# millardjn/rusty_sr

Measured on AMD Instinct MI355X. Metric: output megapixels/sec at 3x upscale (BASELINE '4x'; reference factor is hard-wired 3), higher is better.
Workload: dtype f32

## Files before the change

rusty_sr_amd/csrc/sr_api.cpp:

```cpp
#include <hip/hip_runtime.h>

#include <algorithm>
#include <cmath>
#include <cstdio>
#include <cstdlib>
#include <chrono>
#include <cstring>
#include <new>
#include <string>
#include <thread>
#include <vector>

#include "../../include/srhip.h"
#include "../../include/srhip_experimental.h"
#include "sr_kernels.h"
#include "sr_internal.h"

namespace {

struct ParamLayout {
    size_t conv0, f_bias, f_activ, exp_bias, l_bias[3], l_activ[3], conv1, conv2, conv3, conv5, conv6, conv7, conv8,
        conv9, conv10, end;
    int E;
    explicit ParamLayout(int f) {
// ... 54 lines not shown
                                const int rr = c / 8, h = (c / 4) % 2, e = c % 4;
                                dst[base + (size_t)(2 * ts + rr) * 256 + (h * 32 + j) * 4 + e] = src[c];
                            } else {
                                _Float16 hi, lo;
                                split_half_host(src[c], hi, lo);
                                const int h = c / 8, e = c % 8;
                                hp[ts * 512 + (h * 32 + j) * 8 + e] = hi;
                                hp[1024 + ts * 512 + (h * 32 + j) * 8 + e] = lo;
                            }
                        }
                    }
                }
            }
}

void pack_steps_h16(std::vector<float>& dst, const float* w, int ks) {
    const int nt = ks * ks, np = (nt - 1) / 2;
    auto chunk = [&](int tap_a, int half_a, int tap_b, int half_b) {
        const size_t base = dst.size();
        dst.resize(base + kChunk, 0.0f);
        _Float16* hp = (_Float16*)(dst.data() + base);
        for (int ch = 0; ch < 2; ++ch)
            for (int lane = 0; lane < 64; ++lane) {
                const int g = lane >> 4, o = 16 * ch + (lane & 15);
                const int t = (g >> 1) ? tap_b : tap_a, half = (g >> 1) ? half_b : half_a;
                const int tap = (t % ks) * ks + t / ks;
                for (int e = 0; e < 8; ++e) {
                    _Float16 hi, lo;
                    split_half_host(w[((size_t)o * nt + tap) * 32 + 16 * half + 8 * (g & 1) + e], hi, lo);
                    hp[(ch * 64 + lane) * 8 + e] = hi;
// ... 143 lines not shown
    if (!out) return SR_E_INVALID;
    *out = nullptr;
    if (graph != SR_GRAPH_SR_NET && graph != SR_GRAPH_BILINEAR && graph != SR_GRAPH_DOWNSAMPLE) return SR_E_INVALID;
    if (graph == SR_GRAPH_SR_NET ? (factor < 2 || factor > 4) : factor != SR_FACTOR) return SR_E_FACTOR;
    if (n_params != (graph == SR_GRAPH_SR_NET ? ParamLayout(factor).end : 0)) return SR_E_PARAM_COUNT;
    if (graph == SR_GRAPH_SR_NET && !params) return SR_E_INVALID;
    int ndev = 0;
    if (hipGetDeviceCount(&ndev) != hipSuccess || ndev <= 0) return SR_E_NO_DEVICE;
    if (device < 0 || device >= ndev) return SR_E_INVALID;
    sr_ctx* c = new (std::nothrow) sr_ctx();
    if (!c) return SR_E_NOMEM;
    sr_device_guard restore_device;
    c->device = device;
    c->graph = graph;
    c->factor = factor;
    static const char* const kSwitch[12][2] = {{"th", "SRHIP_TH"}, {"pipe", "SRHIP_PIPE"}, {"bw", "SRHIP_BW"}, {"tail", "SRHIP_TAIL"},
                                               {"bands", "SRHIP_BANDS"}, {"geo", "SRHIP_GEO"}, {"rows", "SRHIP_ROWS"}, {"fork", "SRHIP_FORK"},
                                               {"forkshare", "SRHIP_FORKSHARE"}, {"forkmin", "SRHIP_FORKMIN"}, {"forktune", "SRHIP_FORKTUNE"}, {"halo", "SRHIP_HALO"}};
    for (const auto& sw : kSwitch)
        if (const char* e = getenv(sw[1])) (void)sr_set_experiment(c, sw[0], e);
    {
        unsigned long long hsh = 1469598103934665603ull;
        const unsigned char* pb = (const unsigned char*)params;
        for (size_t i = 0; i < n_params * sizeof(float); ++i) { hsh ^= pb[i]; hsh *= 1099511628211ull; }
        c->params_hash = hsh;
    }
    const bool trace = getenv("SRHIP_TRACE") != nullptr;
    auto t_last = std::chrono::steady_clock::now();
    auto mark = [&](const char* what) {
        if (!trace) return;
        const auto now = std::chrono::steady_clock::now();
// ... 43 lines not shown
            auto conv = [&](const float* wp, int ks) { if (h16) pack_steps_h16(w, wp, ks); else pack_steps(w, wp, ks, 1, split != 0, ident); };
            auto exp3 = [&](const float* wp) { pack_steps(w, wp, 3, expand_tiles(factor), split != 0, expand); };
            size_t* off = split ? c->off_wh : c->off_w;
            w.clear(); conv(params + L.conv1, 5);
            off[1] = push(w);
            w.clear(); conv(params + L.conv2, 5); conv(params + L.conv5, 3);
            off[2] = push(w);
            w.clear(); conv(params + L.conv3, 5); conv(params + L.conv6, 3); conv(params + L.conv8, 3);
            off[3] = push(w);
            w.clear();
            exp3(params + L.conv7); exp3(params + L.conv9); exp3(params + L.conv10);
            if (split) pack_lin_split(w, factor);
            else pack_lin(w, factor);
            off[4] = push(w);
        }
        const size_t boff[4] = {L.f_bias, L.l_bias[0], L.l_bias[1], L.l_bias[2]};
        const size_t aoff[4] = {L.f_activ, L.l_activ[0], L.l_activ[1], L.l_activ[2]};
        for (int s = 0; s < 4; ++s) c->off_bias[s] = push(vec32(boff[s], 32));
        for (int s = 0; s < 4; ++s) c->off_beta[s] = push(vec32(aoff[s], 32));
        {
            std::vector<float> eb((size_t)expand_tiles(factor) * 32, 0.0f);
            for (int nt = 0; nt < expand_tiles(factor); ++nt)
                for (int j = 0; j < 32; ++j) {
                    const int ch = expand_channel(factor, nt, j);
                    if (ch >= 0) eb[nt * 32 + j] = params[L.exp_bias + ch];
                }
            c->off_bias[4] = push(eb);
        }
        for (size_t k = L.conv1; k < L.end && c->split_ok; ++k) c->split_ok = std::fabs(params[k]) < 65504.0f;
        for (size_t k = L.conv0; k < L.conv0 + 2400 && c->split_ok; ++k) c->split_ok = std::fabs(params[k]) < 65504.0f;
// ... 89 lines not shown
    } else if (!strcmp(key, "tail")) {
        c->env_tail = *v ? (float)atof(v) : -1.0f;
    } else if (!strcmp(key, "fork")) {
        c->env_fork = *v ? atoi(v) : -1;
    } else if (!strcmp(key, "forkshare")) {
        c->fork_share = *v ? std::min(0.9, std::max(0.1, atof(v))) : 0.5;
    } else if (!strcmp(key, "forkmin")) {
        c->fork_min_rounds = *v ? atof(v) : 3.5;
    } else if (!strcmp(key, "forktune")) {
        c->fork_autotune = strcmp(v, "0") != 0;
        sr_device_guard restore_device;
        (void)hipSetDevice(c->device);
        sr_fork_tune_clear(c);
    } else if (!strcmp(key, "halo")) {
        c->layer_halos = !strcmp(v, "layers");
    } else if (!strcmp(key, "bw")) {
        c->env_bw = *v ? atoi(v) : -1;
    } else {
        return SR_E_INVALID;
    }
    return SR_OK;
}

int sr_get_experiment(sr_ctx* c, const char* key, char* buf, size_t cap) {
    if (!c || !key || !buf || cap == 0) return SR_E_INVALID;
    std::string out;
    if (!strcmp(key, "forktune")) {
        char line[160];
        for (const auto& t : c->fork_tune) {
            snprintf(line, sizeof line, "%dx%d+%d+%d %s %s %s %.4f %.4f\n", t.H, t.W, t.top, t.bot, t.precision == SR_PRECISION_F32 ? "f32" : "split_f16",
// ... 121 lines not shown
int StackJob::prepare() {
    static const int margin[5] = {5, 3, 2, 1, 0};
    tiles_x = (W + 31) / 32;
    const int rc = ensure_features(c, *ws, n, H, W, tiles_x, s);
    if (rc != SR_OK) return rc;
    const int cus = c->cus > 0 ? c->cus : 256;
    const int resident = 2 * cus;
    const bool planar = c->precision == SR_PRECISION_SPLIT_F16;
    for (int k = 0; k < 4; ++k) feat[k] = ws->d_feat[k] + (planar ? (size_t)kFeatPad * ws->pitch * 32 + kFeatPad * 4 : ((size_t)kFeatPad * ws->pitch + kFeatPad) * 32);
    for (int st = 0; st < 5; ++st) {
        Launch& l = L[st];
        l.y0 = layers ? top : std::max(0, top - margin[st]);
        l.y1 = layers ? bot : std::min(H, bot + margin[st]);
        const int rows = l.y1 - l.y0;
        const long tiles8 = (long)n * tiles_x * ((rows + 7) / 8);
        const int forced = (st == 4 && c->factor == 4 && c->precision == SR_PRECISION_SPLIT_F16) ? 4 : c->env_th[st];
        const bool small_launch = tiles8 < 2L * resident;
        const bool split = c->precision == SR_PRECISION_SPLIT_F16;
        const bool one_small_round = small_launch && (long)n * tiles_x * ((rows + 3) / 4) <= resident;
        l.pipe = st > 0 && c->env_pipe != 0 && (c->env_pipe == 2 || !small_launch || split || (st >= 2 && one_small_round));
        l.ty8 = (rows + 7) / 8; l.ty4 = 0;
        if (forced == 4 || (!forced && small_launch && (!split || tiles8 < cus))) {
            l.ty8 = 0; l.ty4 = (rows + 3) / 4;
        } else if (!forced && l.pipe && !small_launch) {
            const double rounds = (double)tiles8 / resident;
            float tail = c->env_tail;
            if (tail < 0.0f) tail = (!split && rounds >= 3.0 && !forked && st != 4) ? 1.0f : 0.0f;
            if (tail > 0.0f) {
                const long per_row = (long)n * tiles_x;
                const int want = (int)((tail * resident + per_row - 1) / per_row);
                l.ty8 = std::max(0, (rows - 4 * want) / 8);
                l.ty4 = std::max(0, (rows - 8 * l.ty8 + 3) / 4);
            }
        }
        if (!forced && l.pipe && !small_launch && !split && l.ty4 == 0 && (double)tiles8 / resident >= 3.0 && rows % 8 >= 1 && rows % 8 <= 4) {
            l.ty8 = rows / 8; l.ty4 = 1;
        }
// ... 46 lines not shown
        HIPCHK(c, hipStreamWaitEvent(s, gate->ready, 0));
        if (mark && gate->mark[1]) HIPCHK(c, hipEventRecord(gate->mark[1], s));
        if (lo >= hi) return rows(y0, y1);
        rc = rows(y0, lo);
        return rc != SR_OK ? rc : rows(hi, y1);
    }
    StageArgs a{};
    float* f = feat[0]; float* l1 = feat[1]; float* l2 = feat[2]; float* l3 = feat[3];
    a.pitch = ws->pitch; a.img_stride = ws->img_stride;
    switch (st) {
        case 1: a.src[0] = f; a.dst = l1; break;
        case 2: a.src[0] = f; a.src[1] = l1; a.dst = l2; break;
        case 3: a.src[0] = f; a.src[1] = l1; a.src[2] = l2; a.dst = l3; break;
        case 4: a.src[0] = l1; a.src[1] = l2; a.src[2] = l3; a.img = d_img; a.out = d_out; break;
    }
    a.wpack = P + (c->precision ? c->off_wh[st] : c->off_w[st]); a.bias = P + c->off_bias[st];
    a.beta = st < 4 ? P + c->off_beta[st] : nullptr;
    a.H = H; a.W = W; a.img_ch = img_ch;
    a.y_begin = y0; a.y_end = y1; a.tiles_x = tiles_x;
    a.n_img = n; a.queue = ws->d_queue + st * 8; a.domain = c->d_domain;
    a.grid[0] = make_tile_grid(8, y0, l.ty8, tiles_x, n, bw);
    a.grid[1] = make_tile_grid(4, y0 + 8 * l.ty8, l.ty4, tiles_x, n, bw);
    if (l.pipe) HIPCHK(c, sr_launch_stage_pipe(st, c->factor, a, c->precision, l.grid, img_u8, out_u8, s));
    else HIPCHK(c, sr_launch_stage(st, c->factor, a, l.th, c->precision, l.grid, img_u8, out_u8, s));
    return SR_OK;
}

}

int sr_run_stack(sr_ctx* c, const void* d_img, bool img_u8, int img_ch, int n, int H, int W, int halo_top,
                 int halo_bot, void* d_out, bool out_u8, hipStream_t s, int slot, const sr_halo_gate* gate) {
    if (!c || !d_img || !d_out || slot < 0 || slot > 1) return SR_E_INVALID;
    sr_device_guard restore_device;
    if (n <= 0 || H <= 0 || W <= 0) return SR_E_INVALID;
    if (img_u8 && img_ch != 3 && img_ch != 4) return SR_E_INVALID;
    if (c->graph != SR_GRAPH_SR_NET) {
        if (halo_top || halo_bot || gate) return SR_E_INVALID;
        if (c->graph == SR_GRAPH_DOWNSAMPLE && (H < 3 || W < 3)) return SR_E_INVALID;
        if (img_u8 != out_u8) return SR_E_INVALID;
// ... 744 lines not shown
```

rusty_sr_amd/csrc/sr_internal.h:

```cpp
#pragma once
#include <hip/hip_runtime.h>

#include <cstdint>
#include <string>
#include <utility>
#include <vector>

#include "../../include/srhip.h"

struct sr_ctx {
    int device = 0;
    int cus = 0, clock_mhz = 0;
    char name[128] = {0};
    hipStream_t stream = nullptr;
    float* d_params = nullptr;
    void* d_qtab = nullptr;
    size_t off_w0 = 0, off_w0h = 0, off_w[5] = {0}, off_wh[5] = {0}, off_bias[5] = {0}, off_beta[5] = {0};
    int precision = 0;
    bool split_ok = true;
    int* h_domain = nullptr;
    int* d_domain = nullptr;
    int domain_fallbacks = 0;
    bool dev_fault = false;
    int graph = SR_GRAPH_SR_NET;
    int factor = SR_FACTOR;
    struct Workspace {
        float* d_feat[4] = {nullptr, nullptr, nullptr, nullptr};
        size_t feat_cap_px = 0;
        int geo_n = 0, geo_h = 0, geo_w = 0;
        int pitch = 0; long img_stride = 0;
        int* d_queue = nullptr;
    } ws[2];
// ... 153 lines not shown
```

rusty_sr_amd/csrc/sr_kernels.h:

```cpp
#pragma once
#include <hip/hip_runtime.h>
#include <stdint.h>

struct TileDiv {
    uint32_t m, s;
};
inline TileDiv make_tile_div(uint32_t d) {
    TileDiv r{1u, 0u};
    while ((1u << r.s) < d) ++r.s;
    r.m = (uint32_t)(((uint64_t)1 << 32) * (((uint64_t)1 << r.s) - d) / d + 1);
    return r;
}

struct Conv0Args {
    const void* img;
    const float* wpack;
    const void* wpack_split;
    const float* bias;
    const float* beta;
    float* dst;
    int H, W, img_ch;
    int pitch;
    long img_stride;
    int y_begin, y_end;
// ... 59 lines not shown
    long total_px;
};
hipError_t sr_launch_clear_borders(const ClearArgs& a, hipStream_t s);

struct AuxArgs {
    const void* img;
    void* out;
    int n, H, W, img_ch;
    const void* qtab;
};
hipError_t sr_aux_build_tables(void** d_tab);
hipError_t sr_launch_aux(int graph, const AuxArgs& a, bool img_u8, bool out_u8, hipStream_t s);

hipError_t sr_launch_conv0(const Conv0Args& a, int th, int prec, int nblk, bool img_u8, hipStream_t s);
hipError_t sr_launch_stage(int stage, int factor, const StageArgs& a, int th, int prec, int nblk, bool img_u8, bool out_u8,
                           hipStream_t s);
hipError_t sr_launch_stage_pipe(int stage, int factor, const StageArgs& a, int prec, int grid, bool img_u8, bool out_u8,
                                hipStream_t s);
```

rusty_sr_amd/csrc/sr_kernels.hip:

```cpp
#include <hip/hip_runtime.h>
#include <stddef.h>
#include <stdint.h>

#include <mutex>
#include <set>
#include <type_traits>
#include <utility>

#include "sr_kernels.h"

#pragma clang fp contract(off)

typedef float f32x2 __attribute__((ext_vector_type(2)));
struct f32p { float x, y; };
__device__ __forceinline__ f32p operator+(f32p a, f32p b) { return f32p{a.x + b.x, a.y + b.y}; }
__device__ __forceinline__ f32p operator-(f32p a, f32p b) { return f32p{a.x - b.x, a.y - b.y}; }
__device__ __forceinline__ f32p operator*(f32p a, f32p b) { return f32p{a.x * b.x, a.y * b.y}; }
__device__ __forceinline__ f32p p_fma(f32p a, f32p b, f32p c) { return f32p{__builtin_fmaf(a.x, b.x, c.x), __builtin_fmaf(a.y, b.y, c.y)}; }
__device__ __forceinline__ void store_map8(char* p, uint32_t a, uint32_t b) { *(uint2*)p = make_uint2(a, b); }
typedef float f32x4 __attribute__((ext_vector_type(4)));
typedef float f32x16 __attribute__((ext_vector_type(16)));
typedef _Float16 f16x8 __attribute__((ext_vector_type(8)));
typedef _Float16 f16x2 __attribute__((ext_vector_type(2)));

// ... 498 lines not shown
                __builtin_amdgcn_sched_barrier(0);
                mfma(cur, nt);
                __builtin_amdgcn_sched_barrier(0);
                cur = nxt;
            }
        }
        const bool last = p == NP - 1 && nt == NTN - 1;
        sm.template end_step<0>(last);
        if (!last) load(nxt, nt + 1 < NTN ? p : p + 1, 0, sm.slot());
        if (((p * NTN + nt) * 4 + 3) % NTN == 0) sm.piece(((p * NTN + nt) * 4 + 3) / NTN);
        __builtin_amdgcn_sched_barrier(0);
        mfma(cur, nt);
        __builtin_amdgcn_sched_barrier(0);
        cur = nxt;
      }
    }
}

template <int TWH, int PS, int LO, int KS, int T, int NTN, typename Stream>
__device__ __forceinline__ void half_steps_h(f32x16 (&accm)[NTN * T], f32x16 (&accx)[NTN * T], const char* hb, const char* ring,
                                             Stream& sm, int wave, int lane) {
    constexpr int NT = KS * KS, NP = (NT + 1) / 2;
    const int i = lane & 31, h = lane >> 5;
    const int wlane = (h * 32 + i) * 16;
    const char* abase = hb + h * PS + ((wave * T) * TWH + i) * 16;
    struct Ops { f16x8 bh[2], bl[2], ah[2][T], al[2][T]; };
    auto row_id = [](int p, int ts, int m) {
        const int t = 2 * p + ts;
        return t < NT ? (t / KS) * 16 + (t % KS) + m : -1;
    };
// ... 428 lines not shown
                        for (int r = 0; r < 16; r += 2) {
                            uint32_t p0, p1;
                            quant2(r, p0, p1);
                            const int row0 = (r & 3) + 8 * (r >> 2);
                            if (writer && x0 + 4 * h + row0 < a.W) base[row0 * FACTOR] = p0;
                            if (writer && x0 + 4 * h + row0 + 1 < a.W) base[(row0 + 1) * FACTOR] = p1;
                        }
                    }
                }
            }
        }
    }
    return stores;
}

template <int N>
struct __attribute__((packed, aligned(4))) DwordRun { uint32_t w[N]; };
template <int N>
__device__ __forceinline__ void store_run_n(char* o, const uint32_t* w) {
    DwordRun<N> r;
#pragma unroll
    for (int k = 0; k < N; ++k) r.w[k] = w[k];
    *(DwordRun<N>*)o = r;
}
__device__ __forceinline__ void store_run_dwords(char* o, const uint32_t* w, int n) {
    if (n == 1) store_run_n<1>(o, w);
    else if (n == 2) store_run_n<2>(o, w);
    else if (n == 3) store_run_n<3>(o, w);
    else if (n == 4) store_run_n<4>(o, w);
    else if (n == 6) store_run_n<6>(o, w);
// ... 176 lines not shown
__device__ __forceinline__ int queue_slot(int x, int nbig, int nsmall, int idx) {
    int start, count;
    run_of_xcd(x, nbig, start, count);
    if (idx < count) return start + idx;
    idx -= count;
    run_of_xcd(x, nsmall, start, count);
    return idx < count ? nbig + start + idx : -1;
}
__device__ __forceinline__ int queue_total(int x, int nbig, int nsmall) {
    int start, cb, cs;
    run_of_xcd(x, nbig, start, cb);
    run_of_xcd(x, nsmall, start, cs);
    return cb + cs;
}
__device__ __forceinline__ int queue_first(int block, int nbig, int nsmall) { return queue_slot(block & 7, nbig, nsmall, block >> 3); }
template <int TH, int NSRC, int KS0, bool FINAL, bool IMG_U8, bool OUT_U8, int PREC, int FACTOR = 3>
__global__ __launch_bounds__(256, 2) void conv_stage_kernel(StageArgs a) {
    __builtin_amdgcn_s_setprio(3);
    constexpr int NW = 4, T = TH / NW;
    constexpr int NTN = FINAL ? (FACTOR * FACTOR + 9) / 10 : 1;
    using G0 = TileGeom<TH, KS0>;
    extern __shared__ __attribute__((aligned(16))) char smem[];
    char* tile = smem;
    char* ring = smem + 8 * G0::PLANE;

    const int tid = threadIdx.x, lane = tid & 63;
    const int wave = __builtin_amdgcn_readfirstlane(tid >> 6);
    const int i = lane & 31;
    constexpr bool H16 = kH16<PREC, FINAL>;
    constexpr int NTAPS = H16 ? KS0 * KS0 + (NSRC - 1) * 9
                              : 2 * ((KS0 * KS0 + 1) / 2 + (NSRC - 1) * 5) * NTN;
    const TileGrid& grid = a.grid[TH == 8 ? 0 : 1];
    float bias[NTN];
#pragma unroll
    for (int nt = 0; nt < NTN; ++nt) bias[nt] = a.bias[nt * 32 + i];
    const float beta = FINAL ? 0.f : a.beta[i];

    TileOffsets<TH, KS0, NW> off0;
    TileOffsets<TH, 3, NW> off3;
    off0.template init<PREC>(a.pitch, wave, lane);
    if constexpr (NSRC >= 2) off3.template init<PREC>(a.pitch, wave, lane);
    int n, tx, ty;
    tile_coords(grid, a.tiles_x, xcd_remap(blockIdx.x, gridDim.x), n, tx, ty);
    const int x0 = tx * kTW, y0 = grid.y0 + ty * TH;
#pragma unroll
// ... 9 lines not shown
            if constexpr (PREC == 1) accx[m][r] = 0.f;
        }
    f32x4 qm[H16 ? T : 1][2][2], qx[H16 ? T : 1][2][2];
    f32x4 bias2[2], beta2[2];
    if constexpr (H16) {
#pragma unroll
        for (int ch = 0; ch < 2; ++ch) {
            bias2[ch] = *(const f32x4*)(a.bias + 16 * ch + 4 * (lane >> 4));
            beta2[ch] = *(const f32x4*)(a.beta + 16 * ch + 4 * (lane >> 4));
        }
#pragma unroll
        for (int m = 0; m < T; ++m)
#pragma unroll
            for (int k = 0; k < 4; ++k) { qm[m][k >> 1][k & 1] = bias2[k & 1]; qx[m][k >> 1][k & 1] = f32x4{0.f, 0.f, 0.f, 0.f}; }
    }
    int gtap = 0, slot = 0;
    auto taps = [&](auto ks_tag) {
        constexpr int KS = decltype(ks_tag)::value;
        if constexpr (H16) source_steps_h16<TH, KS, T>(qm, qx, tile, ring, a.wpack, gtap, slot, NTAPS, wave, lane);
        else source_steps<TH, KS, T, NTN, PREC>(acc, accx, tile, ring, a.wpack, gtap, slot, NTAPS, wave, lane);
    };
    ring_barrier<0>();
    __builtin_amdgcn_s_setprio(0);
    taps(std::integral_constant<int, KS0>{});
    if constexpr (NSRC >= 2) {
        __builtin_amdgcn_s_setprio(3);
        stage_tile<TH, 3, PREC, NW>(tile, a.src[1], off3, a.img_stride, a.pitch, n, y0, x0, wave, lane);
        ring_barrier<0>();
        __builtin_amdgcn_s_setprio(0);
        taps(std::integral_constant<int, 3>{});
    }
    if constexpr (NSRC >= 3) {
        __builtin_amdgcn_s_setprio(3);
        stage_tile<TH, 3, PREC, NW>(tile, a.src[2], off3, a.img_stride, a.pitch, n, y0, x0, wave, lane);
        ring_barrier<0>();
        __builtin_amdgcn_s_setprio(0);
        taps(std::integral_constant<int, 3>{});
    }
    __builtin_amdgcn_s_setprio(3);
    if constexpr (FINAL)
        lin_taps<TH, T, IMG_U8, NW * 64, NTN, PREC, FACTOR>(acc, accx, tile, ring, a, a.wpack + (size_t)NTAPS * kChunkFloats, n, y0, x0, wave, lane, tid);
    uint32_t dom = 0;
    if constexpr (H16) {
        stage_epilogue_h16<T>(a, qm, qx, beta2, n, x0, y0, wave, lane, dom);
    } else if constexpr (FINAL && PREC == 1) {
        f32x4 fbias[NTN][4];
#pragma unroll
        for (int nt = 0; nt < NTN; ++nt)
#pragma unroll
            for (int k = 0; k < 4; ++k) fbias[nt][k] = *(const f32x4*)(a.bias + 32 * nt + 16 * (lane >> 5) + 4 * k);
        stage_epilogue_final_t<T, NTN, OUT_U8, FACTOR>(a, acc, accx, fbias, n, x0, y0, wave, lane);
    } else {
        static_assert(PREC == 0, "the split-half mode's tiles have epilogues of their own");
        stage_epilogue<TH, T, NTN, FINAL, OUT_U8, FACTOR>(a, acc, bias, beta, n, x0, y0, wave, lane);
    }
    if constexpr (PREC == 1 && !FINAL) domain_report(dom, a.domain);
}

// ... 260 lines not shown
    }
    __device__ __forceinline__ void piece(int g) {
        if (g < HalfTile<KSN>::G::NG && g < rq.ng) {
            htn.stage_one(g, rq.origin, rq.dst);
            st.tile_seq = ++st.issued;
        }
    }
    __device__ __forceinline__ int slot() const { return st.slot; }
    template <int EXTRA> __device__ __forceinline__ void end_step(bool last) {
        if (last) last_step_hook();
        if (last && mailbox) queue_publish(a, xcd, wave, lane, st, qs, mailbox);
        step_advance<EXTRA>(st, last, PREC == 1 && gs0 + step_no <= kRingAhead);
    }
};

template <int NSRC, int KS0, bool FINAL, bool IMG_U8, bool OUT_U8, int PREC, int FACTOR = 3>
__global__ __launch_bounds__(256, 2) void conv_stage_pipe_kernel(StageArgs a) {
    __builtin_amdgcn_s_setprio(3);
    constexpr int NTN = FINAL ? (FACTOR * FACTOR + 9) / 10 : 1;
    using H0 = HalfTile<KS0>;
    using H3 = HalfTile<3>;
    constexpr int HB = H0::BYTES;
    constexpr int NH = 2 * NSRC;
    constexpr bool H16 = kH16<PREC, FINAL>;
    constexpr int NSTEPS = H16 ? KS0 * KS0 + (NSRC - 1) * 9
                               : 2 * (H0::STEPS + (NSRC - 1) * H3::STEPS) * NTN;
    extern __shared__ __attribute__((aligned(16))) char smem[];
    char* ring = smem + 2 * HB;
    volatile int* s_next = (volatile int*)(ring + kRingBytes);
    float* s_wlin = (float*)(ring + kRingBytes + 16);
    float* s_lut = s_wlin + 9 * NTN * 128;
    constexpr bool kLinOwn = FINAL && NTN == 1;
    float* s_xown = s_lut + 256;
    const uint32_t lds0 = lds_addr(smem);

    const int tid = threadIdx.x, lane = tid & 63;
    const int wave = __builtin_amdgcn_readfirstlane(tid >> 6);
    const int i = lane & 31;
    const int nbig = a.grid[0].ntiles, nsmall = a.grid[1].ntiles;
    const int xcd = blockIdx.x & 7;
// ... 85 lines not shown
        f32x4 qm[H16 ? T : 1][2][2], qx[H16 ? T : 1][2][2];
        if constexpr (H16) {
#pragma unroll
            for (int m = 0; m < T; ++m)
#pragma unroll
                for (int k = 0; k < 4; ++k) { qm[m][k >> 1][k & 1] = bias2[k & 1]; qx[m][k >> 1][k & 1] = f32x4{0.f, 0.f, 0.f, 0.f}; }
        }
        constexpr bool QUAD = FINAL && PREC == 0 && T == 2;
        QuadAcc qa[QUAD ? NTN : 1];
        if constexpr (QUAD) {
#pragma unroll
            for (int nt = 0; nt < NTN; ++nt)
#pragma unroll
                for (int g = 0; g < 8; ++g) qa[nt][g] = f32x4{0.f, 0.f, 0.f, 0.f};
        }
        QueueState qs{0u, 0u, 0, 0, -1};
        if (!single) queue_pull_async(a, xcd, wave, lane, st, qs);
        st.have_next = false;
        LinPrefetch<IMG_U8, TH> linpx;
        auto do_half = [&](auto jc) {
            constexpr int j = decltype(jc)::value;
            constexpr int src = j >> 1;
            constexpr int KSJ = src == 0 ? KS0 : 3;
            constexpr int KSN = (j + 1 < NH) ? (((j + 1) >> 1) == 0 ? KS0 : 3) : KS0;
            const uint32_t other = lds0 + ((j + 1) & 1) * HB;
            const char* hb = smem + (j & 1) * HB;
            if constexpr (j == 1) {
                const int next = single ? -1 : __builtin_amdgcn_readfirstlane(*s_next);
                st.have_next = next >= 0;
                if (st.have_next) coords(next, nn, nx0, ny0, nsmall_tile);
            }
            HalfRequest rq;
            if constexpr (j + 1 < NH)
                rq = HalfRequest{T == 2 ? HalfTile<KSN>::G::NG : HalfTile<KSN>::NG_SMALL,
                                 HalfTile<KSN>::template origin_of<PREC>(a.src[(j + 1) >> 1], (j + 1) & 1, a.img_stride, a.pitch, n, y0, x0, wave),
                                 HalfTile<KSN>::plane_of(other, wave)};
            else
                rq = HalfRequest{!st.have_next ? 0 : nsmall_tile ? HalfTile<KSN>::NG_SMALL : HalfTile<KSN>::G::NG,
                                 HalfTile<KSN>::template origin_of<PREC>(a.src[0], 0, a.img_stride, a.pitch, nn, ny0, nx0, wave),
                                 HalfTile<KSN>::plane_of(other, wave)};
            if constexpr (FINAL && j == (kLinOwn ? NH - 2 : NH - 1)) linpx.issue(a, n, y0, x0, tid, st);
            const HalfTile<KSN>* htn;
            if constexpr (KSN == KS0) htn = (const HalfTile<KSN>*)&h0; else htn = (const HalfTile<KSN>*)&h3;
            using GJ = TileGeom<8, KSJ>;
            constexpr int PAIRS_J = (KSJ * KSJ - 1) / 2;
            constexpr int STEPS_J = H16 ? PAIRS_J + (j & 1) : HalfTile<KSJ>::STEPS * NTN;
            constexpr int GS0 = H16 ? (src == 0 ? 0 : KS0 * KS0 + (src - 1) * 9) + (j & 1) * PAIRS_J
                                    : (j == 0 ? 0 : j == 1 ? H0::STEPS : 2 * H0::STEPS + (j - 2) * H3::STEPS) * NTN;
            constexpr int LIN_LO_J = LinPrefetch<IMG_U8, TH>::NPIX * 8;
            auto lin_store = [&]() {
                if constexpr (kLinOwn && j == NH - 2) {
                    if constexpr (PREC == 1) linpx.store_split((char*)s_xown, LIN_LO_J, (const uint32_t*)s_lut, 4.0f * FACTOR * FACTOR, tid, st);
                    else linpx.store(s_xown, s_lut, tid, st);
                    asm volatile("s_waitcnt lgkmcnt(0)" ::: "memory");
                }
            };
            PipeStream<PREC, KSN, decltype(lin_store)> sm{st, rq, *htn, a, ring_lds, wbase, GS0, wave, lane, (j == 0 && !single) ? s_next : nullptr, xcd, qs, STEPS_J > 3 ? STEPS_J - 3 : 0, 0, lin_store};
            if constexpr (QUAD) half_steps_f32<GJ::TWH, GJ::PLANE, KSJ, T, NTN, true, FACTOR>(qa, hb, ring, sm, wave, lane);
            else if constexpr (PREC == 0) half_steps_f32<GJ::TWH, GJ::PLANE, KSJ, T, NTN>(acc, hb, ring, sm, wave, lane);
            else if constexpr (H16) half_steps_h16<GJ::TWH, GJ::PLANE, 2, KSJ, T, (j & 1) != 0, -HB>(qm, qx, hb, ring, sm, wave, lane);
            else half_steps_h<GJ::TWH, GJ::PLANE, 2, KSJ, T, NTN>(acc, accx, hb, ring, sm, wave, lane);
        };
        do_half(std::integral_constant<int, 0>{});
        do_half(std::integral_constant<int, 1>{});
        if constexpr (NH > 2) { do_half(std::integral_constant<int, 2>{}); do_half(std::integral_constant<int, 3>{}); }
        if constexpr (NH > 4) { do_half(std::integral_constant<int, 4>{}); do_half(std::integral_constant<int, 5>{}); }
        if constexpr (FINAL) {
            constexpr int LIN_LO = LinPrefetch<IMG_U8, TH>::NPIX * 8;
            float* s_x = kLinOwn ? s_xown : (float*)(smem + HB);
            if constexpr (!kLinOwn) {
                if constexpr (PREC == 1) linpx.store_split((char*)s_x, LIN_LO, (const uint32_t*)s_lut, 4.0f * FACTOR * FACTOR, tid, st);
                else linpx.store(s_x, s_lut, tid, st);
                asm volatile("s_waitcnt lgkmcnt(0)" ::: "memory");
// ... 3 lines not shown
            if constexpr (PREC == 1) lin_mfma_h<TH, T, NTN>(acc, accx, (const char*)s_x, LIN_LO, (const f16x8*)s_wlin, wave, lane);
            else if constexpr (QUAD) lin_mfma_quad<NTN, FACTOR>(qa, s_x, s_wlin, wave, lane);
            else lin_mfma<TH, T, NTN>(acc, s_x, s_wlin, wave, lane);
            if constexpr (!kLinOwn) {
                asm volatile("s_waitcnt lgkmcnt(0)" ::: "memory");
                __builtin_amdgcn_s_barrier();
                asm volatile("" ::: "memory");
            }
        }
        int stores;
        if constexpr (H16) stores = stage_epilogue_h16<T>(a, qm, qx, beta2, n, x0, y0, wave, lane, dom);
        else if constexpr (QUAD) stores = stage_epilogue_quad<NTN, OUT_U8, FACTOR>(a, qa, qbias, n, x0, y0, wave, lane);
        else if constexpr (kFinalT) stores = stage_epilogue_final_t<T, NTN, OUT_U8, FACTOR>(a, acc, accx, fbias, n, x0, y0, wave, lane);
        else {
            float* scratch = FINAL ? nullptr : (float*)(smem + ((NH - 1) & 1) * HB + wave * H0::G::PLANE);
            stores = stage_epilogue<TH, T, NTN, FINAL, OUT_U8, FACTOR>(a, acc, bias, beta, n, x0, y0, wave, lane, scratch);
        }
        if constexpr (PREC == 1) st.issued += stores;
    };

    constexpr bool kBigTiles = !(FINAL && FACTOR == 4 && PREC == 1);
    int budget = nbig + nsmall;
    while (true) {
        if constexpr (kBigTiles) {
            if (small) tile_body(std::integral_constant<int, 1>{});
            else tile_body(std::integral_constant<int, 2>{});
        } else {
            if (!small) __builtin_trap();
            tile_body(std::integral_constant<int, 1>{});
        }
        if (!st.have_next) break;
// ... 76 lines not shown
    if (e != hipSuccess) return e;
    {
        std::lock_guard<std::mutex> lock(mu);
        const auto key = std::make_pair((const void*)kern, dev);
        if (!configured.count(key)) {
            e = hipFuncSetAttribute((const void*)kern, hipFuncAttributeMaxDynamicSharedMemorySize, (int)lds);
            if (e != hipSuccess) return e;
            configured.insert(key);
        }
    }
    hipLaunchKernelGGL(kern, dim3(nblk), dim3(kThreads), lds, s, a);
    return hipGetLastError();
}

template <int TH, int PREC>
static hipError_t launch_stage_t(int stage, int factor, const StageArgs& a, int nblk, bool img_u8, bool out_u8,
                                 hipStream_t s) {
    switch (stage) {
        case 1: return launch_with_lds(conv_stage_kernel<TH, 1, 5, false, false, false, PREC>, a, nblk, stage_lds_bytes<TH, 5>(), s);
        case 2: return launch_with_lds(conv_stage_kernel<TH, 2, 5, false, false, false, PREC>, a, nblk, stage_lds_bytes<TH, 5>(), s);
        case 3: return launch_with_lds(conv_stage_kernel<TH, 3, 5, false, false, false, PREC>, a, nblk, stage_lds_bytes<TH, 5>(), s);
        case 4:
#define SR_FINAL(F)                                                                                                          \
            if (img_u8 && out_u8) return launch_with_lds(conv_stage_kernel<TH, 3, 3, true, true, true, PREC, F>, a, nblk, stage_lds_bytes<TH, 3>(), s); \
            if (!img_u8 && !out_u8) return launch_with_lds(conv_stage_kernel<TH, 3, 3, true, false, false, PREC, F>, a, nblk, stage_lds_bytes<TH, 3>(), s); \
            return hipErrorInvalidValue;
            if (factor == 3) { SR_FINAL(3) }
            if (factor == 2) { SR_FINAL(2) }
            if (factor == 4) { SR_FINAL(4) }
#undef SR_FINAL
            return hipErrorInvalidValue;
        default: return hipErrorInvalidValue;
    }
}

template <int PREC>
static hipError_t launch_stage_pipe_t(int stage, int factor, const StageArgs& a, int grid, bool img_u8, bool out_u8, hipStream_t s) {
    constexpr size_t lds5 = 2 * (size_t)HalfTile<5>::BYTES + kRingBytes + 16;
    constexpr size_t lds3_1 = 2 * (size_t)HalfTile<3>::BYTES + kRingBytes + 16 + 9 * 128 * sizeof(float) + 256 * sizeof(float) + 10 * 34 * 16;
    constexpr size_t lds3_2 = 2 * (size_t)HalfTile<3>::BYTES + kRingBytes + 16 + 9 * 2 * 128 * sizeof(float) + 256 * sizeof(float);
    static_assert(lds3_1 <= 80 * 1024 && lds3_2 <= 80 * 1024, "two workgroups per CU");
    const size_t lds3 = factor == 4 ? lds3_2 : lds3_1;
    switch (stage) {
        case 1: return launch_with_lds(conv_stage_pipe_kernel<1, 5, false, false, false, PREC>, a, grid, lds5, s);
        case 2: return launch_with_lds(conv_stage_pipe_kernel<2, 5, false, false, false, PREC>, a, grid, lds5, s);
        case 3: return launch_with_lds(conv_stage_pipe_kernel<3, 5, false, false, false, PREC>, a, grid, lds5, s);
        case 4:
#define SR_FINAL(F)                                                                                                          \
            if (img_u8 && out_u8) return launch_with_lds(conv_stage_pipe_kernel<3, 3, true, true, true, PREC, F>, a, grid, lds3, s); \
            if (!img_u8 && !out_u8) return launch_with_lds(conv_stage_pipe_kernel<3, 3, true, false, false, PREC, F>, a, grid, lds3, s); \
            return hipErrorInvalidValue;
            if (factor == 3) { SR_FINAL(3) }
            if (factor == 2) { SR_FINAL(2) }
            if (factor == 4) { SR_FINAL(4) }
#undef SR_FINAL
            return hipErrorInvalidValue;
    }
    return hipErrorInvalidValue;
}
hipError_t sr_launch_stage_pipe(int stage, int factor, const StageArgs& a, int prec, int grid, bool img_u8, bool out_u8, hipStream_t s) {
    return prec == 0 ? launch_stage_pipe_t<0>(stage, factor, a, grid, img_u8, out_u8, s)
                     : launch_stage_pipe_t<1>(stage, factor, a, grid, img_u8, out_u8, s);
}

hipError_t sr_launch_stage(int stage, int factor, const StageArgs& a, int th, int prec, int nblk, bool img_u8,
                           bool out_u8, hipStream_t s) {
    if (prec == 0)
        return th == 8 ? launch_stage_t<8, 0>(stage, factor, a, nblk, img_u8, out_u8, s)
                       : launch_stage_t<4, 0>(stage, factor, a, nblk, img_u8, out_u8, s);
    return th == 8 ? launch_stage_t<8, 1>(stage, factor, a, nblk, img_u8, out_u8, s)
                   : launch_stage_t<4, 1>(stage, factor, a, nblk, img_u8, out_u8, s);
}
```

Measured before the change: 4780.

## Use Winograd F(2,3)-style transform for stage-1 5x5 conv in f32 mode

Adds a Winograd-style minimal-filtering path for the first 5x5 convolution stage in exact f32 precision. The 5-tap rows are split into a 3-tap and a 2-tap part, so the filter transform runs on the host and the input transform is done with packed adds before the MFMAs, reducing the MFMA count per output pair. A dedicated epilogue applies the output transform, bias and activation. It is enabled by default and can be switched off through SRHIP_WINO. Risks include small numerical differences and a changed tile-shape choice, since the small-launch 4-row path is skipped when the new path is on.

```diff
diff --git a/rusty_sr_amd/csrc/sr_api.cpp b/rusty_sr_amd/csrc/sr_api.cpp
--- a/rusty_sr_amd/csrc/sr_api.cpp
+++ b/rusty_sr_amd/csrc/sr_api.cpp
@@ -92,6 +92,28 @@
             }
 }
 
+void pack_steps_wino(std::vector<float>& dst, const float* w) {
+    constexpr int kGroups = 5 * 7 * 2, kSteps = (kGroups + 3) / 4;
+    for (int half = 0; half < 2; ++half) {
+        const size_t base = dst.size();
+        dst.resize(base + (size_t)kSteps * kChunk, 0.0f);
+        for (int g = 0; g < kGroups; ++g) {
+            const int rr = g & 1, k = (g >> 1) % 7, ky = (g >> 1) / 7;
+            float* chunk = dst.data() + base + (size_t)(g / 4) * kChunk + (g % 4) * 256;
+            for (int j = 0; j < 32; ++j)
+                for (int h = 0; h < 2; ++h)
+                    for (int e = 0; e < 4; ++e) {
+                        const int c = 16 * half + 8 * rr + 4 * h + e;
+                        auto tap = [&](int kx) { return (double)w[((size_t)j * 25 + ky * 5 + kx) * 32 + c]; };
+                        const double g0 = k < 4 ? tap(0) : 0.0, g1 = k < 4 ? tap(1) : tap(3), g2 = k < 4 ? tap(2) : tap(4);
+                        const int pos = k < 4 ? k : k - 3;
+                        const double v = pos == 0 ? g0 : pos == 1 ? (g0 + g1 + g2) * 0.5 : pos == 2 ? (g0 - g1 + g2) * 0.5 : g2;
+                        chunk[(h * 32 + j) * 4 + e] = (float)v;
+                    }
+        }
+    }
+}
+
 void pack_steps_h16(std::vector<float>& dst, const float* w, int ks) {
     const int nt = ks * ks, np = (nt - 1) / 2;
     auto chunk = [&](int tap_a, int half_a, int tap_b, int half_b) {
@@ -265,7 +287,7 @@
     c->device = device;
     c->graph = graph;
     c->factor = factor;
-    static const char* const kSwitch[12][2] = {{"th", "SRHIP_TH"}, {"pipe", "SRHIP_PIPE"}, {"bw", "SRHIP_BW"}, {"tail", "SRHIP_TAIL"},
+    static const char* const kSwitch[13][2] = {{"wino", "SRHIP_WINO"}, {"th", "SRHIP_TH"}, {"pipe", "SRHIP_PIPE"}, {"bw", "SRHIP_BW"}, {"tail", "SRHIP_TAIL"},
                                                {"bands", "SRHIP_BANDS"}, {"geo", "SRHIP_GEO"}, {"rows", "SRHIP_ROWS"}, {"fork", "SRHIP_FORK"},
                                                {"forkshare", "SRHIP_FORKSHARE"}, {"forkmin", "SRHIP_FORKMIN"}, {"forktune", "SRHIP_FORKTUNE"}, {"halo", "SRHIP_HALO"}};
     for (const auto& sw : kSwitch)
@@ -339,6 +361,8 @@
             else pack_lin(w, factor);
             off[4] = push(w);
         }
+        w.clear(); pack_steps_wino(w, params + L.conv1);
+        c->off_wino1 = push(w);
         const size_t boff[4] = {L.f_bias, L.l_bias[0], L.l_bias[1], L.l_bias[2]};
         const size_t aoff[4] = {L.f_activ, L.l_activ[0], L.l_activ[1], L.l_activ[2]};
         for (int s = 0; s < 4; ++s) c->off_bias[s] = push(vec32(boff[s], 32));
@@ -458,6 +482,8 @@
         sr_fork_tune_clear(c);
     } else if (!strcmp(key, "halo")) {
         c->layer_halos = !strcmp(v, "layers");
+    } else if (!strcmp(key, "wino")) {
+        c->wino = strcmp(v, "0") != 0;
     } else if (!strcmp(key, "bw")) {
         c->env_bw = *v ? atoi(v) : -1;
     } else {
@@ -609,13 +635,14 @@
         l.y1 = layers ? bot : std::min(H, bot + margin[st]);
         const int rows = l.y1 - l.y0;
         const long tiles8 = (long)n * tiles_x * ((rows + 7) / 8);
+        const bool wino8 = st == 1 && c->precision == SR_PRECISION_F32 && c->wino;
         const int forced = (st == 4 && c->factor == 4 && c->precision == SR_PRECISION_SPLIT_F16) ? 4 : c->env_th[st];
         const bool small_launch = tiles8 < 2L * resident;
         const bool split = c->precision == SR_PRECISION_SPLIT_F16;
         const bool one_small_round = small_launch && (long)n * tiles_x * ((rows + 3) / 4) <= resident;
         l.pipe = st > 0 && c->env_pipe != 0 && (c->env_pipe == 2 || !small_launch || split || (st >= 2 && one_small_round));
         l.ty8 = (rows + 7) / 8; l.ty4 = 0;
-        if (forced == 4 || (!forced && small_launch && (!split || tiles8 < cus))) {
+        if (forced == 4 || (!forced && small_launch && !wino8 && (!split || tiles8 < cus))) {
             l.ty8 = 0; l.ty4 = (rows + 3) / 4;
         } else if (!forced && l.pipe && !small_launch) {
             const double rounds = (double)tiles8 / resident;
@@ -692,15 +719,16 @@
         case 3: a.src[0] = f; a.src[1] = l1; a.src[2] = l2; a.dst = l3; break;
         case 4: a.src[0] = l1; a.src[1] = l2; a.src[2] = l3; a.img = d_img; a.out = d_out; break;
     }
-    a.wpack = P + (c->precision ? c->off_wh[st] : c->off_w[st]); a.bias = P + c->off_bias[st];
+    const bool wino = st == 1 && c->precision == SR_PRECISION_F32 && c->wino;
+    a.wpack = P + (c->precision ? c->off_wh[st] : wino ? c->off_wino1 : c->off_w[st]); a.bias = P + c->off_bias[st];
     a.beta = st < 4 ? P + c->off_beta[st] : nullptr;
     a.H = H; a.W = W; a.img_ch = img_ch;
     a.y_begin = y0; a.y_end = y1; a.tiles_x = tiles_x;
     a.n_img = n; a.queue = ws->d_queue + st * 8; a.domain = c->d_domain;
     a.grid[0] = make_tile_grid(8, y0, l.ty8, tiles_x, n, bw);
     a.grid[1] = make_tile_grid(4, y0 + 8 * l.ty8, l.ty4, tiles_x, n, bw);
-    if (l.pipe) HIPCHK(c, sr_launch_stage_pipe(st, c->factor, a, c->precision, l.grid, img_u8, out_u8, s));
-    else HIPCHK(c, sr_launch_stage(st, c->factor, a, l.th, c->precision, l.grid, img_u8, out_u8, s));
+    if (l.pipe) HIPCHK(c, sr_launch_stage_pipe(st, c->factor, a, c->precision, l.grid, img_u8, out_u8, wino, s));
+    else HIPCHK(c, sr_launch_stage(st, c->factor, a, l.th, c->precision, l.grid, img_u8, out_u8, wino, s));
     return SR_OK;
 }
 
diff --git a/rusty_sr_amd/csrc/sr_internal.h b/rusty_sr_amd/csrc/sr_internal.h
--- a/rusty_sr_amd/csrc/sr_internal.h
+++ b/rusty_sr_amd/csrc/sr_internal.h
@@ -16,6 +16,8 @@
     float* d_params = nullptr;
     void* d_qtab = nullptr;
     size_t off_w0 = 0, off_w0h = 0, off_w[5] = {0}, off_wh[5] = {0}, off_bias[5] = {0}, off_beta[5] = {0};
+    size_t off_wino1 = 0;
+    bool wino = true;
     int precision = 0;
     bool split_ok = true;
     int* h_domain = nullptr;
diff --git a/rusty_sr_amd/csrc/sr_kernels.h b/rusty_sr_amd/csrc/sr_kernels.h
--- a/rusty_sr_amd/csrc/sr_kernels.h
+++ b/rusty_sr_amd/csrc/sr_kernels.h
@@ -97,6 +97,6 @@
 
 hipError_t sr_launch_conv0(const Conv0Args& a, int th, int prec, int nblk, bool img_u8, hipStream_t s);
 hipError_t sr_launch_stage(int stage, int factor, const StageArgs& a, int th, int prec, int nblk, bool img_u8, bool out_u8,
-                           hipStream_t s);
+                           bool wino, hipStream_t s);
 hipError_t sr_launch_stage_pipe(int stage, int factor, const StageArgs& a, int prec, int grid, bool img_u8, bool out_u8,
-                                hipStream_t s);
+                                bool wino, hipStream_t s);
diff --git a/rusty_sr_amd/csrc/sr_kernels.hip b/rusty_sr_amd/csrc/sr_kernels.hip
--- a/rusty_sr_amd/csrc/sr_kernels.hip
+++ b/rusty_sr_amd/csrc/sr_kernels.hip
@@ -536,6 +536,76 @@
         __builtin_amdgcn_sched_barrier(0);
         cur = nxt;
       }
+    }
+}
+
+constexpr int kWinoGroups = 5 * 7 * 2;
+constexpr int kWinoSteps = (kWinoGroups + 3) / 4;
+constexpr int wino_acc(int k) { return k < 4 ? k : k - 3; }
+constexpr int wino_ca(int k) { return k == 0 ? 0 : k == 1 ? 1 : k == 2 ? 2 : k == 3 ? 1 : k == 4 ? 3 : k == 5 ? 4 : 3; }
+constexpr int wino_cb(int k) { return k == 0 ? 2 : k == 1 ? 2 : k == 2 ? 1 : k == 3 ? 3 : k == 4 ? 4 : k == 5 ? 3 : 5; }
+constexpr bool wino_add(int k) { return k == 1 || k == 4; }
+
+template <bool ADD>
+__device__ __forceinline__ void wino_u4(f32x2 x0, f32x2 y0, f32x2 x1, f32x2 y1, f32x2& u0, f32x2& u1) {
+    if constexpr (ADD)
+        asm("v_pk_add_f32 %0, %2, %3\n\tv_pk_add_f32 %1, %4, %5\n\ts_nop 1"
+            : "=&v"(u0), "=&v"(u1) : "v"(x0), "v"(y0), "v"(x1), "v"(y1));
+    else
+        asm("v_pk_add_f32 %0, %2, %3 neg_lo:[0,1] neg_hi:[0,1]\n\tv_pk_add_f32 %1, %4, %5 neg_lo:[0,1] neg_hi:[0,1]\n\ts_nop 1"
+            : "=&v"(u0), "=&v"(u1) : "v"(x0), "v"(y0), "v"(x1), "v"(y1));
+}
+
+template <int TWH, int PS, int T, typename Stream>
+__device__ __forceinline__ void half_steps_wino(f32x16 (&acc)[4], const char* hb, const char* ring, Stream& sm, int wave, int lane) {
+    static_assert(TWH >= kTW + 4, "a pair reads six pixels from its first halo column on");
+    const int i = lane & 31, h = lane >> 5;
+    const int wlane = (h * 32 + i) * 16;
+    const int row = wave * T + (T == 2 ? i >> 4 : 0);
+    const char* abase = hb + h * PS + (row * TWH + 2 * (i & 15)) * 16;
+    struct Ops { f32x4 x, y, b; };
+    auto load = [&](Ops& o, int g, int sl) {
+        const int rr = g & 1, k = (g >> 1) % 7, ky = (g >> 1) / 7;
+        const char* ab = abase + rr * 2 * PS + ky * TWH * 16;
+        o.b = *(const f32x4*)(ring + sl * 4096 + wlane + (g & 3) * 1024);
+        o.x = *(const f32x4*)(ab + wino_ca(k) * 16);
+        o.y = *(const f32x4*)(ab + wino_cb(k) * 16);
+    };
+    auto mfma = [&](const Ops& o, int g) {
+        const int k = (g >> 1) % 7;
+        const f32x2 x0 = {o.x[0], o.x[1]}, x1 = {o.x[2], o.x[3]}, y0 = {o.y[0], o.y[1]}, y1 = {o.y[2], o.y[3]};
+        f32x2 u0, u1;
+        if (wino_add(k)) wino_u4<true>(x0, y0, x1, y1, u0, u1);
+        else wino_u4<false>(x0, y0, x1, y1, u0, u1);
+        const float u[4] = {u0.x, u0.y, u1.x, u1.y};
+#pragma unroll
+        for (int e = 0; e < 4; ++e) acc[wino_acc(k)] = __builtin_amdgcn_mfma_f32_32x32x2f32(u[e], o.b[e], acc[wino_acc(k)], 0, 0, 0);
+    };
+    Ops cur, nxt;
+    load(cur, 0, sm.slot());
+#pragma unroll
+    for (int s = 0; s < kWinoSteps; ++s) {
+        const int ngroups = kWinoGroups - 4 * s < 4 ? kWinoGroups - 4 * s : 4;
+        sm.begin_step();
+#pragma unroll
+        for (int q = 0; q < 3; ++q) {
+            if (q + 1 < ngroups) {
+                load(nxt, 4 * s + q + 1, sm.slot());
+                sm.piece(4 * s + q);
+                __builtin_amdgcn_sched_barrier(0);
+                mfma(cur, 4 * s + q);
+                __builtin_amdgcn_sched_barrier(0);
+                cur = nxt;
+            }
+        }
+        const bool last = s == kWinoSteps - 1;
+        sm.template end_step<0>(last);
+        if (!last) load(nxt, 4 * s + 4, sm.slot());
+        sm.piece(4 * s + 3);
+        __builtin_amdgcn_sched_barrier(0);
+        mfma(cur, 4 * s + ngroups - 1);
+        __builtin_amdgcn_sched_barrier(0);
+        cur = nxt;
     }
 }
 
@@ -994,6 +1064,50 @@
     return stores;
 }
 
+template <int T>
+__device__ __forceinline__ int stage_epilogue_wino(const StageArgs& a, const f32x16 (&acc)[4], float bias, float beta, int n, int x0, int y0,
+                                                   int wave, int lane, float* stage_lds) {
+    const int i = lane & 31, h = lane >> 5;
+    const bool full_x = x0 + kTW <= a.W;
+    int stores = 0;
+#pragma unroll
+    for (int m = 0; m < T; ++m) {
+        const int y = y0 + wave * T + m;
+        if (y >= a.y_end) continue;
+        float* grow = a.dst + ((size_t)n * a.img_stride + (long)y * a.pitch + x0) * 32;
+        float o[16];
+#pragma unroll
+        for (int k = 0; k < 8; k += 2) {
+            const int r = 8 * m + k;
+            const f32x2 m0 = {acc[0][r], acc[0][r + 1]}, m1 = {acc[1][r], acc[1][r + 1]};
+            const f32x2 m2 = {acc[2][r], acc[2][r + 1]}, m3 = {acc[3][r], acc[3][r + 1]};
+            const f32x2 bb = {bias, bias};
+            const f32x2 p0 = belu2(((m0 + m1) + m2) + bb, beta), p1 = belu2(((m1 - m2) - m3) + bb, beta);
+            o[2 * k] = p0.x; o[2 * k + 1] = p1.x; o[2 * k + 2] = p0.y; o[2 * k + 3] = p1.y;
+        }
+        auto pixel = [&](int v) { return 2 * (((v >> 1) & 3) + 8 * (v >> 3) + 4 * h) + (v & 1); };
+        if (full_x && stage_lds) {
+            float* sp = stage_lds + i;
+#pragma unroll
+            for (int v = 0; v < 16; ++v) sp[pixel(v) * 32] = o[v];
+            const f32x4* lp = (const f32x4*)stage_lds + lane;
+            const f32x4 v0 = lp[0], v1 = lp[64], v2 = lp[128], v3 = lp[192];
+            f32x4* gp = (f32x4*)grow + lane;
+            gp[0] = v0; gp[64] = v1; gp[128] = v2; gp[192] = v3;
+            stores += 4;
+        } else if (full_x) {
+#pragma unroll
+            for (int v = 0; v < 16; ++v) grow[pixel(v) * 32 + i] = o[v];
+            stores += 16;
+        } else {
+#pragma unroll
+            for (int v = 0; v < 16; ++v)
+                if (x0 + pixel(v) < a.W) grow[pixel(v) * 32 + i] = o[v];
+        }
+    }
+    return stores;
+}
+
 template <int N>
 struct __attribute__((packed, aligned(4))) DwordRun { uint32_t w[N]; };
 template <int N>
@@ -1200,8 +1314,9 @@
     return cb + cs;
 }
 __device__ __forceinline__ int queue_first(int block, int nbig, int nsmall) { return queue_slot(block & 7, nbig, nsmall, block >> 3); }
-template <int TH, int NSRC, int KS0, bool FINAL, bool IMG_U8, bool OUT_U8, int PREC, int FACTOR = 3>
+template <int TH, int NSRC, int KS0, bool FINAL, bool IMG_U8, bool OUT_U8, int PREC, int FACTOR = 3, bool WINO = false>
 __global__ __launch_bounds__(256, 2) void conv_stage_kernel(StageArgs a) {
+    static_assert(!WINO || (NSRC == 1 && KS0 == 5 && !FINAL && PREC == 0), "WINO: stage 1 of the exact mode");
     __builtin_amdgcn_s_setprio(3);
     constexpr int NW = 4, T = TH / NW;
     constexpr int NTN = FINAL ? (FACTOR * FACTOR + 9) / 10 : 1;
@@ -1214,7 +1329,8 @@
     const int wave = __builtin_amdgcn_readfirstlane(tid >> 6);
     const int i = lane & 31;
     constexpr bool H16 = kH16<PREC, FINAL>;
-    constexpr int NTAPS = H16 ? KS0 * KS0 + (NSRC - 1) * 9
+    constexpr int NTAPS = WINO ? 2 * kWinoSteps
+                        : H16 ? KS0 * KS0 + (NSRC - 1) * 9
                               : 2 * ((KS0 * KS0 + 1) / 2 + (NSRC - 1) * 5) * NTN;
     const TileGrid& grid = a.grid[TH == 8 ? 0 : 1];
     float bias[NTN];
@@ -1254,10 +1370,20 @@
 #pragma unroll
             for (int k = 0; k < 4; ++k) { qm[m][k >> 1][k & 1] = bias2[k & 1]; qx[m][k >> 1][k & 1] = f32x4{0.f, 0.f, 0.f, 0.f}; }
     }
+    f32x16 wacc[WINO ? 4 : 1];
+#pragma unroll
+    for (int p = 0; p < (WINO ? 4 : 1); ++p)
+#pragma unroll
+        for (int r = 0; r < 16; ++r) wacc[p][r] = 0.f;
     int gtap = 0, slot = 0;
     auto taps = [&](auto ks_tag) {
         constexpr int KS = decltype(ks_tag)::value;
-        if constexpr (H16) source_steps_h16<TH, KS, T>(qm, qx, tile, ring, a.wpack, gtap, slot, NTAPS, wave, lane);
+        if constexpr (WINO) {
+            using G = TileGeom<TH, KS>;
+            RingStream sm{ring, a.wpack, gtap, slot, NTAPS, wave, lane};
+#pragma unroll 1
+            for (int half = 0; half < 2; ++half) half_steps_wino<G::TWH, G::PLANE, T>(wacc, tile + half * 4 * G::PLANE, ring, sm, wave, lane);
+        } else if constexpr (H16) source_steps_h16<TH, KS, T>(qm, qx, tile, ring, a.wpack, gtap, slot, NTAPS, wave, lane);
         else source_steps<TH, KS, T, NTN, PREC>(acc, accx, tile, ring, a.wpack, gtap, slot, NTAPS, wave, lane);
     };
     ring_barrier<0>();
@@ -1281,7 +1407,9 @@
     if constexpr (FINAL)
         lin_taps<TH, T, IMG_U8, NW * 64, NTN, PREC, FACTOR>(acc, accx, tile, ring, a, a.wpack + (size_t)NTAPS * kChunkFloats, n, y0, x0, wave, lane, tid);
     uint32_t dom = 0;
-    if constexpr (H16) {
+    if constexpr (WINO) {
+        stage_epilogue_wino<T>(a, wacc, bias[0], beta, n, x0, y0, wave, lane, nullptr);
+    } else if constexpr (H16) {
         stage_epilogue_h16<T>(a, qm, qx, beta2, n, x0, y0, wave, lane, dom);
     } else if constexpr (FINAL && PREC == 1) {
         f32x4 fbias[NTN][4];
@@ -1572,8 +1700,9 @@
     }
 };
 
-template <int NSRC, int KS0, bool FINAL, bool IMG_U8, bool OUT_U8, int PREC, int FACTOR = 3>
+template <int NSRC, int KS0, bool FINAL, bool IMG_U8, bool OUT_U8, int PREC, int FACTOR = 3, bool WINO = false>
 __global__ __launch_bounds__(256, 2) void conv_stage_pipe_kernel(StageArgs a) {
+    static_assert(!WINO || (NSRC == 1 && KS0 == 5 && !FINAL && PREC == 0), "WINO: stage 1 of the exact mode");
     __builtin_amdgcn_s_setprio(3);
     constexpr int NTN = FINAL ? (FACTOR * FACTOR + 9) / 10 : 1;
     using H0 = HalfTile<KS0>;
@@ -1581,7 +1710,8 @@
     constexpr int HB = H0::BYTES;
     constexpr int NH = 2 * NSRC;
     constexpr bool H16 = kH16<PREC, FINAL>;
-    constexpr int NSTEPS = H16 ? KS0 * KS0 + (NSRC - 1) * 9
+    constexpr int NSTEPS = WINO ? 2 * kWinoSteps
+                         : H16 ? KS0 * KS0 + (NSRC - 1) * 9
                                : 2 * (H0::STEPS + (NSRC - 1) * H3::STEPS) * NTN;
     extern __shared__ __attribute__((aligned(16))) char smem[];
     char* ring = smem + 2 * HB;
@@ -1697,6 +1827,11 @@
 #pragma unroll
                 for (int g = 0; g < 8; ++g) qa[nt][g] = f32x4{0.f, 0.f, 0.f, 0.f};
         }
+        f32x16 wacc[WINO ? 4 : 1];
+#pragma unroll
+        for (int p = 0; p < (WINO ? 4 : 1); ++p)
+#pragma unroll
+            for (int r = 0; r < 16; ++r) wacc[p][r] = 0.f;
         QueueState qs{0u, 0u, 0, 0, -1};
         if (!single) queue_pull_async(a, xcd, wave, lane, st, qs);
         st.have_next = false;
@@ -1727,8 +1862,8 @@
             if constexpr (KSN == KS0) htn = (const HalfTile<KSN>*)&h0; else htn = (const HalfTile<KSN>*)&h3;
             using GJ = TileGeom<8, KSJ>;
             constexpr int PAIRS_J = (KSJ * KSJ - 1) / 2;
-            constexpr int STEPS_J = H16 ? PAIRS_J + (j & 1) : HalfTile<KSJ>::STEPS * NTN;
-            constexpr int GS0 = H16 ? (src == 0 ? 0 : KS0 * KS0 + (src - 1) * 9) + (j & 1) * PAIRS_J
+            constexpr int STEPS_J = WINO ? kWinoSteps : H16 ? PAIRS_J + (j & 1) : HalfTile<KSJ>::STEPS * NTN;
+            constexpr int GS0 = WINO ? j * kWinoSteps : H16 ? (src == 0 ? 0 : KS0 * KS0 + (src - 1) * 9) + (j & 1) * PAIRS_J
                                     : (j == 0 ? 0 : j == 1 ? H0::STEPS : 2 * H0::STEPS + (j - 2) * H3::STEPS) * NTN;
             constexpr int LIN_LO_J = LinPrefetch<IMG_U8, TH>::NPIX * 8;
             auto lin_store = [&]() {
@@ -1739,7 +1874,8 @@
                 }
             };
             PipeStream<PREC, KSN, decltype(lin_store)> sm{st, rq, *htn, a, ring_lds, wbase, GS0, wave, lane, (j == 0 && !single) ? s_next : nullptr, xcd, qs, STEPS_J > 3 ? STEPS_J - 3 : 0, 0, lin_store};
-            if constexpr (QUAD) half_steps_f32<GJ::TWH, GJ::PLANE, KSJ, T, NTN, true, FACTOR>(qa, hb, ring, sm, wave, lane);
+            if constexpr (WINO) half_steps_wino<GJ::TWH, GJ::PLANE, T>(wacc, hb, ring, sm, wave, lane);
+            else if constexpr (QUAD) half_steps_f32<GJ::TWH, GJ::PLANE, KSJ, T, NTN, true, FACTOR>(qa, hb, ring, sm, wave, lane);
             else if constexpr (PREC == 0) half_steps_f32<GJ::TWH, GJ::PLANE, KSJ, T, NTN>(acc, hb, ring, sm, wave, lane);
             else if constexpr (H16) half_steps_h16<GJ::TWH, GJ::PLANE, 2, KSJ, T, (j & 1) != 0, -HB>(qm, qx, hb, ring, sm, wave, lane);
             else half_steps_h<GJ::TWH, GJ::PLANE, 2, KSJ, T, NTN>(acc, accx, hb, ring, sm, wave, lane);
@@ -1773,7 +1909,8 @@
         else if constexpr (kFinalT) stores = stage_epilogue_final_t<T, NTN, OUT_U8, FACTOR>(a, acc, accx, fbias, n, x0, y0, wave, lane);
         else {
             float* scratch = FINAL ? nullptr : (float*)(smem + ((NH - 1) & 1) * HB + wave * H0::G::PLANE);
-            stores = stage_epilogue<TH, T, NTN, FINAL, OUT_U8, FACTOR>(a, acc, bias, beta, n, x0, y0, wave, lane, scratch);
+            if constexpr (WINO) stores = stage_epilogue_wino<T>(a, wacc, bias[0], beta, n, x0, y0, wave, lane, scratch);
+            else stores = stage_epilogue<TH, T, NTN, FINAL, OUT_U8, FACTOR>(a, acc, bias, beta, n, x0, y0, wave, lane, scratch);
         }
         if constexpr (PREC == 1) st.issued += stores;
     };
@@ -1880,10 +2017,13 @@
 }
 
 template <int TH, int PREC>
-static hipError_t launch_stage_t(int stage, int factor, const StageArgs& a, int nblk, bool img_u8, bool out_u8,
+static hipError_t launch_stage_t(int stage, int factor, const StageArgs& a, int nblk, bool img_u8, bool out_u8, bool wino,
                                  hipStream_t s) {
     switch (stage) {
-        case 1: return launch_with_lds(conv_stage_kernel<TH, 1, 5, false, false, false, PREC>, a, nblk, stage_lds_bytes<TH, 5>(), s);
+        case 1:
+            if constexpr (PREC == 0)
+                if (wino) return launch_with_lds(conv_stage_kernel<TH, 1, 5, false, false, false, 0, 3, true>, a, nblk, stage_lds_bytes<TH, 5>(), s);
+            return launch_with_lds(conv_stage_kernel<TH, 1, 5, false, false, false, PREC>, a, nblk, stage_lds_bytes<TH, 5>(), s);
         case 2: return launch_with_lds(conv_stage_kernel<TH, 2, 5, false, false, false, PREC>, a, nblk, stage_lds_bytes<TH, 5>(), s);
         case 3: return launch_with_lds(conv_stage_kernel<TH, 3, 5, false, false, false, PREC>, a, nblk, stage_lds_bytes<TH, 5>(), s);
         case 4:
@@ -1901,14 +2041,17 @@
 }
 
 template <int PREC>
-static hipError_t launch_stage_pipe_t(int stage, int factor, const StageArgs& a, int grid, bool img_u8, bool out_u8, hipStream_t s) {
+static hipError_t launch_stage_pipe_t(int stage, int factor, const StageArgs& a, int grid, bool img_u8, bool out_u8, bool wino, hipStream_t s) {
     constexpr size_t lds5 = 2 * (size_t)HalfTile<5>::BYTES + kRingBytes + 16;
     constexpr size_t lds3_1 = 2 * (size_t)HalfTile<3>::BYTES + kRingBytes + 16 + 9 * 128 * sizeof(float) + 256 * sizeof(float) + 10 * 34 * 16;
     constexpr size_t lds3_2 = 2 * (size_t)HalfTile<3>::BYTES + kRingBytes + 16 + 9 * 2 * 128 * sizeof(float) + 256 * sizeof(float);
     static_assert(lds3_1 <= 80 * 1024 && lds3_2 <= 80 * 1024, "two workgroups per CU");
     const size_t lds3 = factor == 4 ? lds3_2 : lds3_1;
     switch (stage) {
-        case 1: return launch_with_lds(conv_stage_pipe_kernel<1, 5, false, false, false, PREC>, a, grid, lds5, s);
+        case 1:
+            if constexpr (PREC == 0)
+                if (wino) return launch_with_lds(conv_stage_pipe_kernel<1, 5, false, false, false, 0, 3, true>, a, grid, lds5, s);
+            return launch_with_lds(conv_stage_pipe_kernel<1, 5, false, false, false, PREC>, a, grid, lds5, s);
         case 2: return launch_with_lds(conv_stage_pipe_kernel<2, 5, false, false, false, PREC>, a, grid, lds5, s);
         case 3: return launch_with_lds(conv_stage_pipe_kernel<3, 5, false, false, false, PREC>, a, grid, lds5, s);
         case 4:
@@ -1924,16 +2067,16 @@
     }
     return hipErrorInvalidValue;
 }
-hipError_t sr_launch_stage_pipe(int stage, int factor, const StageArgs& a, int prec, int grid, bool img_u8, bool out_u8, hipStream_t s) {
-    return prec == 0 ? launch_stage_pipe_t<0>(stage, factor, a, grid, img_u8, out_u8, s)
-                     : launch_stage_pipe_t<1>(stage, factor, a, grid, img_u8, out_u8, s);
+hipError_t sr_launch_stage_pipe(int stage, int factor, const StageArgs& a, int prec, int grid, bool img_u8, bool out_u8, bool wino, hipStream_t s) {
+    return prec == 0 ? launch_stage_pipe_t<0>(stage, factor, a, grid, img_u8, out_u8, wino, s)
+                     : launch_stage_pipe_t<1>(stage, factor, a, grid, img_u8, out_u8, wino, s);
 }
 
 hipError_t sr_launch_stage(int stage, int factor, const StageArgs& a, int th, int prec, int nblk, bool img_u8,
-                           bool out_u8, hipStream_t s) {
+                           bool out_u8, bool wino, hipStream_t s) {
     if (prec == 0)
-        return th == 8 ? launch_stage_t<8, 0>(stage, factor, a, nblk, img_u8, out_u8, s)
-                       : launch_stage_t<4, 0>(stage, factor, a, nblk, img_u8, out_u8, s);
-    return th == 8 ? launch_stage_t<8, 1>(stage, factor, a, nblk, img_u8, out_u8, s)
-                   : launch_stage_t<4, 1>(stage, factor, a, nblk, img_u8, out_u8, s);
-}
+        return th == 8 ? launch_stage_t<8, 0>(stage, factor, a, nblk, img_u8, out_u8, wino, s)
+                       : launch_stage_t<4, 0>(stage, factor, a, nblk, img_u8, out_u8, wino, s);
+    return th == 8 ? launch_stage_t<8, 1>(stage, factor, a, nblk, img_u8, out_u8, wino, s)
+                   : launch_stage_t<4, 1>(stage, factor, a, nblk, img_u8, out_u8, wino, s);
+}
```

Result: faster. 5000, median of 6 (+4.6%).
